# hongsukchoi/Pose2Mesh_RELEASE

Measured on NVIDIA H100. Metric: SMPL meshes/sec, higher is better.
Workload: dtype f32 (wgmma fp16x3 split, fp32 accumulate)

## Files before the change

pose2mesh_release_b200/csrc/cheb_umma.cu:

```cuda
#include <cuda.h>
#include <cuda_fp16.h>
#include <cuda_runtime.h>

#include <algorithm>
#include <cstdlib>
#include <cstring>
#include <vector>

#include "p2m_internal.h"

namespace p2m {

namespace {

constexpr int TILE_M = 128;
constexpr int FC = 32;
constexpr int A_BLOCK_BYTES = TILE_M * 128;
constexpr float W_SCALE = 64.f;
constexpr float W_INV_SCALE = 1.f / 64.f;

struct TileHeader {
  int n_rows;
  int h1;
  int nnz;
// ... 63 lines not shown
}
template <unsigned SLEEP_NS = 200>
__device__ __forceinline__ void mbar_wait_relaxed(uint32_t bar, uint32_t parity, volatile int* abort_flag, int* status,
                                                  int code) {
  if (mbar_try_wait(bar, parity)) return;
  unsigned long long t0 = 0;
  for (unsigned spin = 0;; ++spin) {
#pragma unroll 1
    for (int it = 0; it < 16; ++it) {
      if (mbar_try_wait(bar, parity)) return;
      __nanosleep(SLEEP_NS);
    }
    if (*abort_flag) return;
    if ((spin & 255u) == 255u) {
      const unsigned long long t = global_ns();
      if (t0 == 0) t0 = t;
      else if (t - t0 > MBAR_TIMEOUT_NS) break;
    }
  }
  mbar_timeout(abort_flag, status, code);
}
__device__ __forceinline__ void fence_barrier_init() { asm volatile("fence.mbarrier_init.release.cluster;" ::: "memory"); }
__device__ __forceinline__ void fence_async_proxy() { asm volatile("fence.proxy.async.shared::cta;" ::: "memory"); }

__device__ __forceinline__ void bulk_g2s(uint32_t dst, const void* src, uint32_t bytes, uint32_t bar) {
  asm volatile("cp.async.bulk.shared::cluster.global.mbarrier::complete_tx::bytes [%0], [%1], %2, [%3];" ::"r"(dst),
               "l"(src), "r"(bytes), "r"(bar)
               : "memory");
}
__device__ __forceinline__ void bulk_s2g(void* dst, uint32_t src, uint32_t bytes) {
  asm volatile("cp.async.bulk.global.shared::cta.bulk_group [%0], [%1], %2;" ::"l"(dst), "r"(src), "r"(bytes) : "memory");
}
__device__ __forceinline__ void bulk_commit() { asm volatile("cp.async.bulk.commit_group;" ::: "memory"); }
__device__ __forceinline__ void bulk_wait_read0() { asm volatile("cp.async.bulk.wait_group.read 0;" ::: "memory"); }
__device__ __forceinline__ void bulk_wait0() { asm volatile("cp.async.bulk.wait_group 0;" ::: "memory"); }
__device__ __forceinline__ void cp_async16(uint32_t dst, const void* src) {
  asm volatile("cp.async.cg.shared.global [%0], [%1], 16;" ::"r"(dst), "l"(src) : "memory");
}
__device__ __forceinline__ void cp_async16_zfill(uint32_t dst, const void* src, uint32_t src_bytes) {
  asm volatile("cp.async.cg.shared.global [%0], [%1], 16, %2;" ::"r"(dst), "l"(src), "r"(src_bytes) : "memory");
}
__device__ __forceinline__ void tma_load_2d(uint32_t dst, const CUtensorMap* tm, int c0, int c1, uint32_t bar) {
  asm volatile(
      "cp.async.bulk.tensor.2d.shared::cluster.global.mbarrier::complete_tx::bytes [%0], [%1, {%2, %3}], [%4];" ::"r"(dst),
      "l"(reinterpret_cast<uint64_t>(tm)), "r"(c0), "r"(c1), "r"(bar)
      : "memory");
}
__device__ __forceinline__ void prefetch_l2(const void* ptr) {
  asm volatile("prefetch.global.L2 [%0];" ::"l"(ptr));
}
__device__ __forceinline__ void cp_async_arrive_noinc(uint32_t bar) {
  asm volatile("cp.async.mbarrier.arrive.noinc.shared::cta.b64 [%0];" ::"r"(bar) : "memory");
}
__device__ __forceinline__ void producer_barrier() { asm volatile("bar.sync 1, 512;" ::: "memory"); }
__device__ __forceinline__ float4 lds_f4(uint32_t a) {
  float4 v;
  asm volatile("ld.shared.v4.f32 {%0, %1, %2, %3}, [%4];" : "=f"(v.x), "=f"(v.y), "=f"(v.z), "=f"(v.w) : "r"(a));
  return v;
}
__device__ __forceinline__ float2 lds_f2(uint32_t a) {
  float2 v;
  asm volatile("ld.shared.v2.f32 {%0, %1}, [%2];" : "=f"(v.x), "=f"(v.y) : "r"(a));
  return v;
}
__device__ __forceinline__ uint2 lds_u2(uint32_t a) {
  uint2 v;
  asm volatile("ld.shared.v2.u32 {%0, %1}, [%2];" : "=r"(v.x), "=r"(v.y) : "r"(a));
  return v;
}
__device__ __forceinline__ uint32_t lds_u16(uint32_t a) {
  unsigned short v;
  asm volatile("ld.shared.u16 %0, [%1];" : "=h"(v) : "r"(a));
  return v;
}
__device__ __forceinline__ void sts_f4(uint32_t a, const float4& v) {
  asm volatile("st.shared.v4.f32 [%0], {%1, %2, %3, %4};" ::"r"(a), "f"(v.x), "f"(v.y), "f"(v.z), "f"(v.w) : "memory");
}
__device__ __forceinline__ void sts_f2(uint32_t a, float x, float y) {
  asm volatile("st.shared.v2.f32 [%0], {%1, %2};" ::"r"(a), "f"(x), "f"(y) : "memory");
}
__device__ __forceinline__ void sts_u2(uint32_t a, const uint2& v) {
  asm volatile("st.shared.v2.u32 [%0], {%1, %2};" ::"r"(a), "r"(v.x), "r"(v.y) : "memory");
}
__device__ __forceinline__ void fma4(float4& acc, float w, const float4& x) {
  acc.x = fmaf(w, x.x, acc.x);
  acc.y = fmaf(w, x.y, acc.y);
  acc.z = fmaf(w, x.z, acc.z);
  acc.w = fmaf(w, x.w, acc.w);
}
__device__ __forceinline__ float4 cheb_t2(const float4& g, const float4& x) {
  return make_float4(fmaf(2.f, g.x, -x.x), fmaf(2.f, g.y, -x.y), fmaf(2.f, g.z, -x.z), fmaf(2.f, g.w, -x.w));
}
__device__ __forceinline__ float4 gather_row4(uint32_t ent, uint32_t e, uint32_t e1, uint32_t rows_q) {
  float4 acc0 = make_float4(0.f, 0.f, 0.f, 0.f), acc1 = acc0;
  for (; e + 3 < e1; e += 4) {
    const uint2 a0 = lds_u2(ent + e * 8), a1 = lds_u2(ent + e * 8 + 8), a2 = lds_u2(ent + e * 8 + 16),
                a3 = lds_u2(ent + e * 8 + 24);
    const float4 x0 = lds_f4(rows_q + a0.x), x1 = lds_f4(rows_q + a1.x), x2 = lds_f4(rows_q + a2.x),
                 x3 = lds_f4(rows_q + a3.x);
    fma4(acc0, __uint_as_float(a0.y), x0);
    fma4(acc1, __uint_as_float(a1.y), x1);
    fma4(acc0, __uint_as_float(a2.y), x2);
    fma4(acc1, __uint_as_float(a3.y), x3);
  }
  if (e + 1 < e1) {
    const uint2 a0 = lds_u2(ent + e * 8), a1 = lds_u2(ent + e * 8 + 8);
    const float4 x0 = lds_f4(rows_q + a0.x), x1 = lds_f4(rows_q + a1.x);
// ... 55 lines not shown
};
__device__ __forceinline__ void split4(const float4& v, uint2& hi, uint2& lo) {
  __half2 h0 = __floats2half2_rn(v.x, v.y), h1 = __floats2half2_rn(v.z, v.w);
  float2 f0 = __half22float2(h0), f1 = __half22float2(h1);
  __half2 l0 = __floats2half2_rn(v.x - f0.x, v.y - f0.y), l1 = __floats2half2_rn(v.z - f1.x, v.w - f1.y);
  hi.x = *reinterpret_cast<uint32_t*>(&h0);
  hi.y = *reinterpret_cast<uint32_t*>(&h1);
  lo.x = *reinterpret_cast<uint32_t*>(&l0);
  lo.y = *reinterpret_cast<uint32_t*>(&l1);
}

struct KParams {
  const float* x;
  int in_unpool;
  int V, P, fin;
  int n_tiles;
  const unsigned char* meta;
  const int* meta_bytes;
  int meta_stride, max_h1;
  const unsigned char* wpack;
  const float* zero_row;
  EpiDev ep;
  int res_identity;
  const float* t1;
  const float* a_scale;
  long long ldy;
  int y_col0;
  float* y;
  int* status;
  long long* trace;
  int own_table;
  const float* head_wt;
  float* head_z;
  const unsigned char* apack;
  long long wslice_bytes;
  long long wblock_stride;
  int tma;
  CUtensorMap tm_x, tm_t1;
};

#ifdef P2M_UMMA_TRACE
__device__ __forceinline__ void trace_ev(const KParams& p, int role, int& n, int ev) {
  if (p.trace != nullptr && blockIdx.x == 0 && blockIdx.y == 0 && n < 512) {
    p.trace[role * 512 + n] = ((long long)ev << 48) | (clock64() & 0xFFFFFFFFFFFFll);
    ++n;
  }
}
#else
__device__ __forceinline__ void trace_ev(const KParams&, int, int&, int) {}
#endif

constexpr int W_PROD = 16;
constexpr int W_XLOAD = 16, N_XLOAD = 2, W_BLOAD = 18, W_EPI0 = 20;
constexpr int NUM_THREADS2 = 24 * 32;
constexpr int REGS_LAUNCH = 80, REGS_UTIL = 40, REGS_EPI = 120;
static_assert(128 * (REGS_EPI - REGS_LAUNCH) <= 128 * (REGS_LAUNCH - REGS_UTIL), "register pool balance");
static_assert(W_XLOAD % 4 == 0 && W_EPI0 % 4 == 0 && W_EPI0 - W_XLOAD == 4, "setmaxnreg works on aligned warpgroups");

template <int N>
__host__ __device__ constexpr int tile_rows() { return N == 128 ? 64 : TILE_M; }
template <int N, int NS, int XS, int MODE>
__global__ void __launch_bounds__(NUM_THREADS2, 1) k_cheb_conv_umma(const __grid_constant__ KParams p) {
  static_assert(N == 64 || N == 128, "one warpgroup holds the CTA's 128 x 64 or 64 x 128 accumulator in registers");
  constexpr int TM = tile_rows<N>();
  constexpr int RPT = TM / 64;
  constexpr int H = TM / 64;
  constexpr int ER = 16 * H;
  constexpr bool KT1 = (MODE == 1);
  constexpr bool plain = !KT1;
  constexpr bool XDIRECT = KT1 && NS >= 3;
  constexpr int A_BYTES = TM * 128;
  constexpr int B_BLOCK_BYTES = N * 128;
  constexpr int SLOT_BYTES = A_BYTES + B_BLOCK_BYTES;

  extern __shared__ __align__(1024) unsigned char smem_raw[];
  unsigned char* ring = smem_raw;
  float* Xs = reinterpret_cast<float*>(ring + NS * SLOT_BYTES);
  const size_t xs_stage_floats = (XDIRECT && TM == 64) ? 0 : (size_t)TM * FC;
  float* T1s = Xs + XS * xs_stage_floats;
  const size_t t1_stage_floats = (size_t)p.max_h1 * FC;
  unsigned char* meta_s =
      reinterpret_cast<unsigned char*>(T1s + (plain ? 0 : XS) * t1_stage_floats);
  uint64_t* bars = reinterpret_cast<uint64_t*>(meta_s + 2 * (size_t)p.meta_stride);
  uint64_t* b_ab_full = bars;
  uint64_t* b_ab_empty = b_ab_full + NS;
  uint64_t* b_x_full = b_ab_empty + NS;
  uint64_t* b_x_empty = b_x_full + XS;
  uint64_t* b_m_full = b_x_empty + XS;
  uint64_t* b_m_empty = b_m_full + 2;
  uint32_t* flags = reinterpret_cast<uint32_t*>(b_m_empty + 2);
  volatile int* abort_flag = reinterpret_cast<volatile int*>(flags + 1);
  float* ep_mul = reinterpret_cast<float*>(flags + 4);
  float* ep_add = ep_mul + N;
  constexpr int EC = 32;
  constexpr int STG_WARP_BYTES = N == 128 ? 16 * STG_ROW_BYTES : 32 * EC * 4;
  unsigned char* epi_stage =
      reinterpret_cast<unsigned char*>((reinterpret_cast<uintptr_t>(ep_add + N) + 127) & ~(uintptr_t)127);
  int* own_s = reinterpret_cast<int*>(epi_stage + 4 * STG_WARP_BYTES);
  float* head_w_s = reinterpret_cast<float*>(own_s + 4 * 32);
  uint64_t* b_res = reinterpret_cast<uint64_t*>(head_w_s);

  const int tid = threadIdx.x;
  const int warp = tid >> 5;
  const int lane = tid & 31;
  const int n_chunk = p.fin / FC;
  const int n_use = 3 * n_chunk;

  if (tid == 0) {
    for (int s = 0; s < NS; ++s) {
      mbar_init(smem_u32(b_ab_full + s), p.apack != nullptr ? 1 : W_PROD + 1);
      mbar_init(smem_u32(b_ab_empty + s), 4);
    }
    for (int s = 0; s < XS; ++s) {
      mbar_init(smem_u32(b_x_full + s), N_XLOAD * 32 + 1);
      mbar_init(smem_u32(b_x_empty + s), 1);
    }
    for (int s = 0; s < 2; ++s) {
      mbar_init(smem_u32(b_m_full + s), 1);
      mbar_init(smem_u32(b_m_empty + s), 1);
    }
    if (N == 128)
      for (int w = 0; w < 4; ++w) mbar_init(smem_u32(b_res + w), 1);
    *abort_flag = (smem_u32(ring) & 1023u) ? 1 : 0;
    if (*abort_flag) mbar_timeout(abort_flag, p.status, 100);
    fence_barrier_init();
  }
  const float a_scale = p.a_scale ? *p.a_scale : 1.f;
  const int ecol0 = (int)blockIdx.y * N;
  for (int n = threadIdx.x; n < N; n += NUM_THREADS2) {
    const float sc = (p.ep.scale ? p.ep.scale[ecol0 + n] : 1.f) / a_scale;
    const float sh = p.ep.scale ? p.ep.shift[ecol0 + n] : 0.f;
    const float bi = p.ep.bias ? p.ep.bias[ecol0 + n] : 0.f;
    ep_mul[n] = W_INV_SCALE * sc;
    ep_add[n] = fmaf(bi, p.ep.scale ? p.ep.scale[ecol0 + n] : 1.f, sh);
  }
  if (N == 64 && p.head_z != nullptr)
    for (int i = threadIdx.x; i < 64 * 12; i += NUM_THREADS2) head_w_s[i] = p.head_wt[i];
  __syncthreads();

  if (warp >= W_XLOAD && warp < W_EPI0) {
  asm volatile("setmaxnreg.dec.sync.aligned.u32 %0;" ::"n"(REGS_UTIL));
  if (warp >= W_XLOAD && warp < W_XLOAD + N_XLOAD) {
    if (p.apack == nullptr) {
      const int lt = tid - W_XLOAD * 32;
      const int lq = lt & 7, lrg = lt >> 3;
      const int my_tiles = (p.n_tiles - (int)blockIdx.x + (int)gridDim.x - 1) / (int)gridDim.x;
      if (lt == 32 && p.tma) {
        if (!XDIRECT) asm volatile("prefetch.tensormap [%0];" ::"l"(reinterpret_cast<uint64_t>(&p.tm_x)) : "memory");
        if (KT1) asm volatile("prefetch.tensormap [%0];" ::"l"(reinterpret_cast<uint64_t>(&p.tm_t1)) : "memory");
      }
      auto fetch_meta = [&](int itf) {
        const int pat = (blockIdx.x + itf * gridDim.x) % p.P;
        const int m = itf & 1;
        mbar_wait_relaxed(smem_u32(b_m_empty + m), ((itf >> 1) & 1) ^ 1, abort_flag, p.status, 1);
        const int mbytes = p.meta_bytes[pat];
        mbar_arrive_expect_tx(smem_u32(b_m_full + m), mbytes);
        bulk_g2s(smem_u32(meta_s + (size_t)m * p.meta_stride), p.meta + (size_t)pat * p.meta_stride, mbytes,
                 smem_u32(b_m_full + m));
      };
      if (lt == 0 && my_tiles > 0) fetch_meta(0);
      const uint32_t fin_bytes = (uint32_t)p.fin * 4u;
      const int sh = p.in_unpool ? 1 : 0;
      int g2 = 0;
      int ltn = 0;
      for (int it2 = 0; it2 < my_tiles; ++it2) {
        const int tile2 = blockIdx.x + it2 * gridDim.x;
        const long long mesh_row0 = (long long)(tile2 / p.P) * p.V;
        const int m2 = it2 & 1;
        mbar_wait_relaxed(smem_u32(b_m_full + m2), (it2 >> 1) & 1, abort_flag, p.status, 8);
        const unsigned char* mb2 = meta_s + (size_t)m2 * p.meta_stride;
        const TileHeader* hdr2 = reinterpret_cast<const TileHeader*>(mb2);
        const int* halo = reinterpret_cast<const int*>(mb2 + hdr2->off_halo);
        const int h1 = hdr2->h1;
        for (int c2 = 0; c2 < n_chunk; ++c2, ++g2) {
          const int xs2 = g2 % XS;
          mbar_wait_relaxed(smem_u32(b_x_empty + xs2), ((g2 / XS) & 1) ^ 1, abort_flag, p.status, 11);
          if (lt == 0) trace_ev(p, 4, ltn, 1);
          const uint32_t xbar = smem_u32(b_x_full + xs2);
          auto stage_rows = [&](uint32_t dbase, const char* sbase, int first, int n_rows, int shift) {
            for (int i0 = first + lrg; i0 < n_rows; i0 += 32) {
              int v[4];
#pragma unroll
              for (int u = 0; u < 4; ++u) v[u] = (i0 + 8 * u < n_rows) ? halo[i0 + 8 * u] : -2;
#pragma unroll
              for (int u = 0; u < 4; ++u) {
                if (v[u] != -2) {
                  const uint32_t srow = (uint32_t)max(v[u], 0) >> shift;
                  cp_async16_zfill(dbase + (i0 + 8 * u) * 128, sbase + (uint64_t)srow * (uint64_t)fin_bytes,
                                   v[u] >= 0 ? 16u : 0u);
                }
              }
            }
          };
          const char* t1_mesh =
              reinterpret_cast<const char*>(KT1 ? p.t1 + mesh_row0 * p.fin + c2 * FC + lq * 4 : nullptr);
          const char* x_mesh = reinterpret_cast<const char*>(p.x + (mesh_row0 >> sh) * p.fin + c2 * FC + lq * 4);
          const uint32_t t1_dst = smem_u32(T1s + xs2 * t1_stage_floats) + lq * 16;
          const uint32_t x_dst = smem_u32(Xs + xs2 * xs_stage_floats) + lq * 16;
          if (p.tma) {
            if (lt == 32) {
              const int own0 = tile2 * TM;
              mbar_arrive_expect_tx(xbar, (XDIRECT ? 0 : (p.in_unpool ? TM / 2 : TM) * 128) + (KT1 ? TM * 128 : 0));
              if (!XDIRECT)
                tma_load_2d(smem_u32(Xs + xs2 * xs_stage_floats), &p.tm_x, c2 * FC, p.in_unpool ? own0 >> 1 : own0, xbar);
              if (KT1) tma_load_2d(smem_u32(T1s + xs2 * t1_stage_floats), &p.tm_t1, c2 * FC, own0, xbar);
            }
            if (KT1) stage_rows(t1_dst, t1_mesh, TM, h1, 0);
          } else {
            if (KT1) stage_rows(t1_dst, t1_mesh, 0, h1, 0);
            if (!XDIRECT) stage_rows(x_dst, x_mesh, 0, TM, sh);
            if (lt == 32) mbar_arrive(xbar);
          }
          cp_async_arrive_noinc(xbar);
          if (lt == 0) trace_ev(p, 4, ltn, 2);
          if (lt == 0 && c2 == (n_chunk > 1 ? 1 : 0) && it2 + 1 < my_tiles) fetch_meta(it2 + 1);
        }
      }
    }
  } else if (warp == W_BLOAD) {
    if (lane == 0) {
      uint32_t ucnt = 0;
      int tn = 0;
      const int uses = plain ? n_chunk : n_use;
      for (int tile = blockIdx.x; tile < p.n_tiles; tile += gridDim.x) {
        for (int u = 0; u < uses; ++u, ++ucnt) {
          const int s = ucnt % NS;
          const uint32_t par = (ucnt / NS) & 1;
          mbar_wait_relaxed(smem_u32(b_ab_empty + s), par ^ 1, abort_flag, p.status, 4);
          trace_ev(p, 1, tn, 10 + u);
          const unsigned char* wsl = p.wpack + (size_t)blockIdx.y * (size_t)p.wslice_bytes;
          if (p.apack != nullptr) {
            mbar_arrive_expect_tx(smem_u32(b_ab_full + s), B_BLOCK_BYTES + A_BYTES);
            bulk_g2s(smem_u32(ring + s * SLOT_BYTES), p.apack + ((size_t)tile * uses + u) * A_BYTES, A_BYTES,
                     smem_u32(b_ab_full + s));
          } else {
            mbar_arrive_expect_tx(smem_u32(b_ab_full + s), B_BLOCK_BYTES);
          }
          bulk_g2s(smem_u32(ring + s * SLOT_BYTES + A_BYTES), wsl + (size_t)u * (size_t)p.wblock_stride, B_BLOCK_BYTES,
                   smem_u32(b_ab_full + s));
        }
      }
    }
  }
  } else if (warp >= W_EPI0) {
    asm volatile("setmaxnreg.inc.sync.aligned.u32 %0;" ::"n"(REGS_EPI));
    const int wq = warp - W_EPI0;
    constexpr int CPR = EC / 4;
    constexpr int RPI = 32 / CPR;
    const uint32_t stg = smem_u32(epi_stage) + (uint32_t)wq * STG_WARP_BYTES;
    const int prow = lane / CPR, pc = lane % CPR;
    constexpr int NP = ER / RPI;
    int colk[2];
#pragma unroll
    for (int k = 0; k < 2; ++k) colk[k] = (int)(((uint32_t)pc ^ (uint32_t)((k * RPI + prow) & 7)) << 2);
    const int trow = (lane >> 4) * 64 + wq * 16 + (lane & 15);
    const int uses = plain ? n_chunk : n_use;
    uint32_t ucnt = 0;
    int it = 0;
    int etn = 0;
    for (int tile = blockIdx.x; tile < p.n_tiles; tile += gridDim.x, ++it) {
      const int b = tile / p.P, pat = tile - b * p.P;
      const long long mesh0 = (long long)b * p.V;
      int* own_w = own_s + wq * 32;
      {
        int v;
        if (lane >= ER) {
          v = -1;
        } else if (p.own_table) {
          v = __ldg(reinterpret_cast<const int*>(p.meta + (size_t)pat * p.meta_stride + 64) + trow);
        } else {
          v = pat * TM + trow;
          if (v >= p.V) v = -1;
        }
        __syncwarp();
        own_w[lane] = v;
        __syncwarp();
      }
      int own_v[NP];
#pragma unroll
      for (int i = 0; i < NP; ++i) own_v[i] = own_w[i * RPI + prow];
      if (N == 128) {
        if (lane < ER) bulk_wait_read0();
        __syncwarp();
        if (p.ep.res != nullptr && p.res_identity) {
          const uint32_t rbar = smem_u32(b_res + wq);
          const int n_valid = __popc(__ballot_sync(0xFFFFFFFFu, lane < ER && own_w[lane] >= 0));
          if (lane == 0) mbar_arrive_expect_tx(rbar, (uint32_t)n_valid * (N * 4));
          __syncwarp();
          if (lane < ER && own_w[lane] >= 0) {
            const long long r = mesh0 + own_w[lane];
            bulk_g2s(stg + lane * STG_ROW_BYTES, p.ep.res + (p.ep.res_unpool ? (r >> 1) : r) * p.ep.res_F + ecol0, N * 4,
                     rbar);
          }
        }
      }
      if (p.ep.res != nullptr && (N == 64 || !p.res_identity)) {
        const int lpr = ((p.apack != nullptr ? N : p.ep.res_F) * 4 + 127) >> 7;
        for (int j = lane; j < ER * lpr; j += 32) {
          const int rr = j / lpr, ln = j - rr * lpr;
          const int vtx = own_w[rr];
          if (vtx >= 0) {
            const long long r = mesh0 + vtx;
            prefetch_l2(p.ep.res + (p.ep.res_unpool ? (r >> 1) : r) * p.ep.res_F + (p.apack != nullptr ? ecol0 : 0) + ln * 32);
          }
        }
      }
      float acc[2][32];
#pragma unroll
      for (int h = 0; h < 2; ++h)
#pragma unroll
        for (int j = 0; j < 32; ++j) acc[h][j] = 0.f;
      if (wq == 0 && lane == 0) trace_ev(p, 3, etn, 1);
      for (int u = 0; u < uses; ++u, ++ucnt) {
        const uint32_t s = ucnt % NS;
        if (wq == 0 && lane == 0) trace_ev(p, 3, etn, 4);
        mbar_wait(smem_u32(b_ab_full + s), (ucnt / NS) & 1, abort_flag, p.status, 6);
        if (wq == 0 && lane == 0) trace_ev(p, 3, etn, 5);
        const uint32_t a0 = smem_u32(ring + s * SLOT_BYTES);
        wg_fence();
#pragma unroll
        for (int h = 0; h < 2; ++h) {
          const uint64_t da = make_desc_sw128(a0 + (TM == 128 ? (uint32_t)h * (64 * 128) : 0u));
          const uint64_t db = make_desc_sw128(a0 + A_BYTES + (TM == 64 ? (uint32_t)h * (64 * 128) : 0u));
          wgmma_m64n64<0, 0>(acc[h], da + 0, db + 0);
          wgmma_m64n64<0, 0>(acc[h], da + 2, db + 2);
          wgmma_m64n64<0, 0>(acc[h], da + 4, db + 0);
          wgmma_m64n64<0, 0>(acc[h], da + 6, db + 2);
          wgmma_m64n64<0, 0>(acc[h], da + 0, db + 4);
          wgmma_m64n64<0, 0>(acc[h], da + 2, db + 6);
        }
        wg_commit();
        wg_wait0();
        __syncwarp();
        if (lane == 0) mbar_arrive(smem_u32(b_ab_empty + s));
      }
      if (wq == 0 && lane == 0) trace_ev(p, 3, etn, 2);
      auto stage_slab = [&](int cb) {
#pragma unroll
        for (int h = 0; h < H; ++h)
#pragma unroll
          for (int jj = 0; jj < 4; ++jj)
#pragma unroll
            for (int r = 0; r < 2; ++r) {
              const int lr = 16 * h + (lane >> 2) + 8 * r;
              const int cc = 8 * jj + 2 * (lane & 3);
              const int j = 4 * (cb / 8 + jj) + 2 * r;
              sts_f2(stg + lr * (EC * 4) + ((((uint32_t)(cc >> 2)) ^ (uint32_t)(lr & 7)) << 4) + (cc & 3) * 4,
                     acc[h][j], acc[h][j + 1]);
            }
        __syncwarp();
      };
      if (N == 64 && p.head_z != nullptr) {
        float z[12];
#pragma unroll
        for (int j = 0; j < 12; ++j) z[j] = 0.f;
#pragma unroll
        for (int cb = 0; cb < N; cb += 32) {
          stage_slab(cb);
#pragma unroll
          for (int c = 0; c < 8; ++c) {
            const float4 a = lds_f4(stg + lane * (EC * 4) + (((uint32_t)c ^ (uint32_t)(lane & 7)) << 4));
            const float av[4] = {a.x, a.y, a.z, a.w};
#pragma unroll
            for (int e = 0; e < 4; ++e) {
              const int n = cb + 4 * c + e;
              float t = fmaf(av[e], ep_mul[n], ep_add[n]);
              if (p.ep.relu) t = fmaxf(t, 0.f);
              const float4 w0 = *reinterpret_cast<const float4*>(head_w_s + n * 12);
              const float4 w1 = *reinterpret_cast<const float4*>(head_w_s + n * 12 + 4);
              const float4 w2 = *reinterpret_cast<const float4*>(head_w_s + n * 12 + 8);
              z[0] = fmaf(t, w0.x, z[0]); z[1] = fmaf(t, w0.y, z[1]); z[2] = fmaf(t, w0.z, z[2]); z[3] = fmaf(t, w0.w, z[3]);
              z[4] = fmaf(t, w1.x, z[4]); z[5] = fmaf(t, w1.y, z[5]); z[6] = fmaf(t, w1.z, z[6]); z[7] = fmaf(t, w1.w, z[7]);
              z[8] = fmaf(t, w2.x, z[8]); z[9] = fmaf(t, w2.y, z[9]); z[10] = fmaf(t, w2.z, z[10]); z[11] = fmaf(t, w2.w, z[11]);
            }
          }
          __syncwarp();
        }
        if (own_w[lane] >= 0) {
          float4* zr = reinterpret_cast<float4*>(p.head_z + (mesh0 + own_w[lane]) * 12);
          zr[0] = make_float4(z[0], z[1], z[2], z[3]);
          zr[1] = make_float4(z[4], z[5], z[6], z[7]);
          zr[2] = make_float4(z[8], z[9], z[10], z[11]);
        }
      } else if (N == 128) {
        const bool res_id = p.ep.res != nullptr && p.res_identity;
        if (res_id) mbar_wait(smem_u32(b_res + wq), (uint32_t)it & 1u, abort_flag, p.status, 12);
        if (wq == 0 && lane == 0) trace_ev(p, 3, etn, 21);
#pragma unroll
        for (int h = 0; h < 2; ++h)
#pragma unroll
          for (int jg = 0; jg < 8; ++jg) {
            const int n = 64 * h + 8 * jg + 2 * (lane & 3);
            const float2 mu = *reinterpret_cast<const float2*>(ep_mul + n);
            const float2 ad = *reinterpret_cast<const float2*>(ep_add + n);
#pragma unroll
            for (int r = 0; r < 2; ++r) {
              const int j = 4 * jg + 2 * r;
              const uint32_t a = stg + ((lane >> 2) + 8 * r) * STG_ROW_BYTES + n * 4;
              float o0 = fmaf(acc[h][j], mu.x, ad.x), o1 = fmaf(acc[h][j + 1], mu.y, ad.y);
              if (p.ep.relu) {
                o0 = fmaxf(o0, 0.f);
                o1 = fmaxf(o1, 0.f);
              }
              if (res_id) {
                const float2 rv = lds_f2(a);
                o0 += rv.x;
                o1 += rv.y;
              }
              sts_f2(a, o0, o1);
            }
          }
        if (p.ep.res != nullptr && !p.res_identity) {
          __syncwarp();
          const int gn = ecol0 + 4 * lane;
          for (int rr = 0; rr < ER; ++rr) {
            const int vtx = own_w[rr];
            if (vtx >= 0) {
              const long long r = mesh0 + vtx;
              const float* res_row = p.ep.res + (p.ep.res_unpool ? (r >> 1) : r) * p.ep.res_F;
              const uint32_t a = stg + rr * STG_ROW_BYTES + lane * 16;
              const float4 v = lds_f4(a);
              float o[4] = {v.x, v.y, v.z, v.w};
#pragma unroll
              for (int e = 0; e < 4; ++e) {
                const float l = __ldg(p.ep.lam + gn + e);
                o[e] += (1.f - l) * __ldg(res_row + __ldg(p.ep.i0 + gn + e)) + l * __ldg(res_row + __ldg(p.ep.i1 + gn + e));
              }
              sts_f4(a, make_float4(o[0], o[1], o[2], o[3]));
            }
          }
        }
        if (wq == 0 && lane == 0) trace_ev(p, 3, etn, 22);
        fence_async_proxy();
        __syncwarp();
        if (lane < ER) {
          if (own_w[lane] >= 0)
            bulk_s2g(p.y + (mesh0 + own_w[lane]) * p.ldy + p.y_col0 + ecol0, stg + lane * STG_ROW_BYTES, N * 4);
          bulk_commit();
        }
        if (wq == 0 && lane == 0) trace_ev(p, 3, etn, 23);
      } else {
#pragma unroll
        for (int cb = 0; cb < N; cb += 32) {
          stage_slab(cb);
          float4 mu_k[2], ad_k[2];
#pragma unroll
          for (int k = 0; k < 2; ++k) {
            mu_k[k] = *reinterpret_cast<const float4*>(ep_mul + cb + colk[k]);
            ad_k[k] = *reinterpret_cast<const float4*>(ep_add + cb + colk[k]);
          }
#pragma unroll
          for (int i = 0; i < NP; ++i) {
            const int rr = i * RPI + prow;
            const int n = cb + colk[i & 1];
            const int gn = ecol0 + n;
            const float4 a = lds_f4(stg + rr * (EC * 4) + (pc << 4));
            const int vtx = own_v[i];
            if (vtx >= 0) {
              const float4 mu = mu_k[i & 1], ad = ad_k[i & 1];
              float o[4] = {fmaf(a.x, mu.x, ad.x), fmaf(a.y, mu.y, ad.y), fmaf(a.z, mu.z, ad.z), fmaf(a.w, mu.w, ad.w)};
              if (p.ep.relu) {
#pragma unroll
                for (int e = 0; e < 4; ++e) o[e] = fmaxf(o[e], 0.f);
              }
              const long long r = mesh0 + vtx;
              if (p.ep.res != nullptr) {
                const float* res_row = p.ep.res + (p.ep.res_unpool ? (r >> 1) : r) * p.ep.res_F;
                if (p.res_identity) {
                  const float4 rv = __ldg(reinterpret_cast<const float4*>(res_row + gn));
                  o[0] += rv.x; o[1] += rv.y; o[2] += rv.z; o[3] += rv.w;
                } else {
#pragma unroll
                  for (int e = 0; e < 4; ++e) {
                    const float l = __ldg(p.ep.lam + gn + e);
                    o[e] += (1.f - l) * __ldg(res_row + __ldg(p.ep.i0 + gn + e)) + l * __ldg(res_row + __ldg(p.ep.i1 + gn + e));
                  }
                }
              }
              *reinterpret_cast<float4*>(p.y + r * p.ldy + p.y_col0 + gn) = make_float4(o[0], o[1], o[2], o[3]);
            }
          }
          __syncwarp();
        }
      }
    }
    if (N == 128 && lane < ER) bulk_wait0();
  } else {
    if (p.apack == nullptr) {
    const int q = tid & 7;
    const int rg = tid >> 3;
    const uint32_t t1s_a = smem_u32(T1s);
    const uint32_t ring_a = smem_u32(ring);
    const int my_tiles = (p.n_tiles - (int)blockIdx.x + (int)gridDim.x - 1) / (int)gridDim.x;
    const int n_stage = my_tiles * n_chunk;

    uint32_t row[RPT], re[RPT], ent_a = 0;
    int ptn = 0;
    uint32_t slot = 0, spar = 0;
    uint32_t so_f[RPT], so_s[RPT];
#pragma unroll
    for (int ps = 0; ps < RPT; ++ps) row[ps] = re[ps] = so_f[ps] = so_s[ps] = 0;
    const bool odd = (rg & 1) != 0;
    auto next_slot = [&]() {
      if (++slot == (uint32_t)NS) {
        slot = 0;
        spar ^= 1u;
      }
    };

    const int xsh = (p.tma && p.in_unpool) ? 1 : 0;
    const float* xp[RPT];
#pragma unroll
    for (int ps = 0; ps < RPT; ++ps) xp[ps] = nullptr;
    int it = 0, c = -1;
    for (int g = 0; g < n_stage; ++g) {
      if (++c == n_chunk) {
        c = 0;
        ++it;
      }
      const int m = it & 1;
      const int xs = g % XS;
      float4 xd[RPT];
#pragma unroll
      for (int ps = 0; ps < RPT; ++ps) {
        xd[ps] = make_float4(0.f, 0.f, 0.f, 0.f);
        if (XDIRECT && c != 0 && xp[ps]) xd[ps] = __ldg(reinterpret_cast<const float4*>(xp[ps] + c * FC));
      }
      if (tid == 0) trace_ev(p, 0, ptn, 1);
      mbar_wait(smem_u32(b_x_full + xs), (g / XS) & 1, abort_flag, p.status, 9);
      if (tid == 0) trace_ev(p, 0, ptn, 2);

      if (c == 0) {
        mbar_wait(smem_u32(b_m_full + m), (it >> 1) & 1, abort_flag, p.status, 8);
        const unsigned char* mb = meta_s + (size_t)m * p.meta_stride;
        const TileHeader* hdr = reinterpret_cast<const TileHeader*>(mb);
        const uint32_t mb_a = smem_u32(mb);
        const uint32_t rp_a = mb_a + hdr->off_rp, ord2_a = mb_a + hdr->off_ord2;
        ent_a = mb_a + hdr->off_ent;
#pragma unroll
        for (int ps = 0; ps < RPT; ++ps) {
          row[ps] = plain ? (uint32_t)(64 * ps + rg) : lds_u16(ord2_a + 2 * (64 * ps + rg));
          re[ps] = plain ? 0u : (lds_u16(rp_a + 2 * row[ps]) | (lds_u16(rp_a + 2 * row[ps] + 2) << 16));
          const uint32_t i = row[ps];
          const uint32_t a_hi = sw128_off(i, q >> 1) + (q & 1) * 8, a_lo = sw128_off(i, 4 + (q >> 1)) + (q & 1) * 8;
          so_f[ps] = odd ? a_lo : a_hi;
          so_s[ps] = odd ? a_hi : a_lo;
        }
        if (XDIRECT) {
          const int* halo = reinterpret_cast<const int*>(mb + hdr->off_halo);
          const int sh = p.in_unpool ? 1 : 0;
          const long long mesh_row0 = (long long)((blockIdx.x + (unsigned)it * gridDim.x) / (unsigned)p.P) * p.V;
          const float* xm = p.x + (mesh_row0 >> sh) * p.fin + q * 4;
#pragma unroll
          for (int ps = 0; ps < RPT; ++ps) {
            const int v = halo[row[ps]];
            xp[ps] = (v >= 0) ? xm + (size_t)((uint32_t)v >> sh) * (uint32_t)p.fin : nullptr;
            if (xp[ps]) xd[ps] = __ldg(reinterpret_cast<const float4*>(xp[ps]));
          }
        }
      }
      const uint32_t xs_q = smem_u32(Xs + xs * xs_stage_floats) + q * 16;
      const uint32_t t1s_q = t1s_a + (uint32_t)(xs * t1_stage_floats * 4) + q * 16;
      if (plain) {
        const uint32_t s = slot;
        mbar_wait(smem_u32(b_ab_empty + s), spar ^ 1u, abort_flag, p.status, 10);
        const uint32_t ablk = ring_a + s * SLOT_BYTES;
#pragma unroll
        for (int ps = 0; ps < RPT; ++ps) {
          const uint32_t i = ps * 64 + rg;
          float4 v = lds_f4(xs_q + (i >> xsh) * 128);
          v.x *= a_scale; v.y *= a_scale; v.z *= a_scale; v.w *= a_scale;
          uint2 hi, lo;
          split4(v, hi, lo);
          sts_u2(ablk + so_f[ps], odd ? lo : hi);
          sts_u2(ablk + so_s[ps], odd ? hi : lo);
        }
        fence_async_proxy();
        __syncwarp();
        if ((tid & 31) == 0) mbar_arrive(smem_u32(b_ab_full + s));
        next_slot();
        producer_barrier();
        if (tid == 0) mbar_arrive(smem_u32(b_x_empty + xs));
        if (tid == 0 && c == n_chunk - 1) mbar_arrive(smem_u32(b_m_empty + m));
        continue;
      }
      const uint32_t slot0 = slot;
      auto emit = [&](const float4 (&vv)[RPT]) {
        const uint32_t s = slot;
        if (NS < 3) mbar_wait(smem_u32(b_ab_empty + s), spar ^ 1u, abort_flag, p.status, 10);
        const uint32_t ablk = ring_a + s * SLOT_BYTES;
#pragma unroll
        for (int ps = 0; ps < RPT; ++ps) {
          uint2 hi, lo;
          float4 v = vv[ps];
          if (p.a_scale != nullptr) {
            v.x *= a_scale; v.y *= a_scale; v.z *= a_scale; v.w *= a_scale;
          }
          split4(v, hi, lo);
          sts_u2(ablk + so_f[ps], odd ? lo : hi);
          sts_u2(ablk + so_s[ps], odd ? hi : lo);
        }
        if (NS < 3) {
          fence_async_proxy();
          __syncwarp();
          if ((tid & 31) == 0) mbar_arrive(smem_u32(b_ab_full + s));
        }
        next_slot();
      };
      float4 x[RPT], t1v[RPT], t2[RPT];
      if (NS < 3) {
#pragma unroll
        for (int ps = 0; ps < RPT; ++ps) x[ps] = lds_f4(xs_q + (row[ps] >> xsh) * 128);
        emit(x);
#pragma unroll
        for (int ps = 0; ps < RPT; ++ps) t1v[ps] = lds_f4(t1s_q + row[ps] * 128);
        emit(t1v);
#pragma unroll
        for (int ps = 0; ps < RPT; ++ps) t2[ps] = gather_row4(ent_a, re[ps] & 0xFFFFu, re[ps] >> 16, t1s_q);
        if (tid == 0) trace_ev(p, 0, ptn, 6);
#pragma unroll
        for (int ps = 0; ps < RPT; ++ps) t2[ps] = cheb_t2(t2[ps], x[ps]);
        emit(t2);
      } else {
#pragma unroll
        for (int ps = 0; ps < RPT; ++ps) t2[ps] = gather_row4(ent_a, re[ps] & 0xFFFFu, re[ps] >> 16, t1s_q);
#pragma unroll
        for (int ps = 0; ps < RPT; ++ps) x[ps] = XDIRECT ? xd[ps] : lds_f4(xs_q + (row[ps] >> xsh) * 128);
#pragma unroll
        for (int ps = 0; ps < RPT; ++ps) t1v[ps] = lds_f4(t1s_q + row[ps] * 128);
        if (tid == 0) trace_ev(p, 0, ptn, 6);
        {
          uint32_t s2 = slot + 2, p2 = spar;
          if (s2 >= (uint32_t)NS) {
            s2 -= (uint32_t)NS;
            p2 ^= 1u;
          }
          mbar_wait(smem_u32(b_ab_empty + s2), p2 ^ 1u, abort_flag, p.status, 10);
        }
        emit(x);
        emit(t1v);
#pragma unroll
        for (int ps = 0; ps < RPT; ++ps) t2[ps] = cheb_t2(t2[ps], x[ps]);
        emit(t2);
      }
      if (NS >= 3) {
        fence_async_proxy();
        __syncwarp();
        if ((tid & 31) == 0) {
#pragma unroll
          for (int k = 0; k < 3; ++k) mbar_arrive(smem_u32(b_ab_full + (slot0 + k) % NS));
        }
      }
      if (tid == 0) trace_ev(p, 0, ptn, 7);
      producer_barrier();
      if (tid == 0) trace_ev(p, 0, ptn, 8);
      if (tid == 0) mbar_arrive(smem_u32(b_x_empty + xs));
      if (tid == 0 && c == n_chunk - 1) mbar_arrive(smem_u32(b_m_empty + m));
    }
    }
  }
}

struct DwParams {
  const float* x;
  int in_unpool;
  int V, P, fin;
  int n_tiles;
  const unsigned char* meta;
  const int* meta_bytes;
  int meta_stride, max_h1;
  const float* g;
  int fout_total, m_off, m_cols;
  int chunk0;
  const float* a_scale;
  float* dw;
  int* status;
  const float* t1;
  int g_unpool;
  int swap;
  int tma;
  CUtensorMap tm_x, tm_t1;
};

__device__ __forceinline__ uint64_t make_desc_sw128_mn(uint32_t saddr, uint32_t lbo_bytes) {
  uint64_t d = 0;
  d |= (uint64_t)((saddr & 0x3FFFF) >> 4);
  d |= (uint64_t)((lbo_bytes >> 4) & 0x3FFF) << 16;
  d |= (uint64_t)(1024 >> 4) << 32;
  d |= (uint64_t)1 << 62;
  return d;
}

constexpr int DW_NS = 3;
constexpr int DW_G_BYTES = 4 * A_BLOCK_BYTES;

template <int XS>
__global__ void __launch_bounds__(NUM_THREADS2, 1) k_cheb_dw_umma(const __grid_constant__ DwParams p) {
  extern __shared__ __align__(1024) unsigned char smem_raw[];
  unsigned char* ring = smem_raw;
  unsigned char* gblk = ring + DW_NS * A_BLOCK_BYTES;
  float* Xs = reinterpret_cast<float*>(gblk + DW_G_BYTES);
  constexpr size_t xs_stage_floats = (size_t)TILE_M * FC;
  float* T1s = Xs + XS * xs_stage_floats;
  const size_t t1_stage_floats = (size_t)p.max_h1 * FC;
  unsigned char* meta_s = reinterpret_cast<unsigned char*>(T1s + XS * t1_stage_floats);
  uint64_t* bars = reinterpret_cast<uint64_t*>(meta_s + 2 * (size_t)p.meta_stride);
  uint64_t* b_t_full = bars;
// ... 216 lines not shown
        }
        fence_async_proxy();
        __syncwarp();
        if ((tid & 31) == 0) mbar_arrive(smem_u32(b_g_full));
      }
      for (int c = 0; c < n_chunk; ++c, ++gcnt) {
        const int xs = gcnt % XS;
        mbar_wait(smem_u32(b_x_full + xs), (gcnt / XS) & 1, abort_flag, p.status, 29);
        const uint32_t xs_q = smem_u32(Xs + xs * xs_stage_floats) + q * 16;
        const uint32_t t1s_q = t1s_a + (uint32_t)(xs * t1_stage_floats * 4) + q * 16;
        float4 tv[3][2];
        {
          const float4 g0 = gather_row4(ent_a, r0e & 0xFFFFu, r0e >> 16, t1s_q);
          const float4 g1 = gather_row4(ent_a, r1e & 0xFFFFu, r1e >> 16, t1s_q);
          tv[0][0] = lds_f4(xs_q + row0 * 128);
          tv[0][1] = lds_f4(xs_q + row1 * 128);
          tv[1][0] = lds_f4(t1s_q + row0 * 128);
          tv[1][1] = lds_f4(t1s_q + row1 * 128);
          const float4 a = tv[0][0], c2 = tv[0][1];
          tv[2][0] = cheb_t2(g0, a);
          tv[2][1] = cheb_t2(g1, c2);
          if (p.swap) {
#pragma unroll
            for (int k = 0; k < 3; ++k)
#pragma unroll
              for (int ps = 0; ps < 2; ++ps) {
                tv[k][ps].x *= a_scale; tv[k][ps].y *= a_scale; tv[k][ps].z *= a_scale; tv[k][ps].w *= a_scale;
              }
          }
        }
        const uint32_t u0 = ucnt;
#pragma unroll
        for (int k = 0; k < 3; ++k, ++ucnt) {
          const int s = ucnt % DW_NS;
          mbar_wait(smem_u32(b_t_empty + s), ((ucnt / DW_NS) & 1) ^ 1, abort_flag, p.status, 30);
          const uint32_t blk = ring_a + s * A_BLOCK_BYTES + (q & 1) * 8;
#pragma unroll
          for (int ps = 0; ps < 2; ++ps) {
            const uint32_t i = ps ? row1 : row0;
            uint2 hi, lo;
            split4(tv[k][ps], hi, lo);
            const uint32_t a_hi = blk + sw128_off(i, q >> 1), a_lo = blk + sw128_off(i, 4 + (q >> 1));
            const bool odd = (rg & 1) != 0;
            sts_u2(odd ? a_lo : a_hi, odd ? lo : hi);
            sts_u2(odd ? a_hi : a_lo, odd ? hi : lo);
          }
        }
        fence_async_proxy();
        __syncwarp();
        if ((tid & 31) == 0) {
#pragma unroll
          for (int k = 0; k < 3; ++k) mbar_arrive(smem_u32(b_t_full + (u0 + k) % DW_NS));
        }
        producer_barrier();
        if (tid == 0) {
          mbar_arrive(smem_u32(b_x_empty + xs));
          if (c == n_chunk - 1) mbar_arrive(smem_u32(b_m_empty + m));
        }
      }
    }
  }
}

struct T1Params {
  const float* x;
  int in_unpool;
  int V, P, fin;
  const unsigned char* meta;
  const int* meta_bytes;
  int meta_stride, max_h1;
  float* t1;
};

template <int T1_STAGES>
__global__ void __launch_bounds__(512, 2) k_cheb_t1(const T1Params p) {
  extern __shared__ __align__(16) unsigned char smem_t1[];
  unsigned char* meta_s = smem_t1;
  float* Xs = reinterpret_cast<float*>(smem_t1 + p.meta_stride);
  const size_t stage_floats = (size_t)p.max_h1 * FC;
  const int tid = threadIdx.x, q = tid & 7, rg = tid >> 3;
  const int tile = blockIdx.x;
  const int b = tile / p.P, pat = tile - b * p.P;
  const long long mesh_row0 = (long long)b * p.V;
  {
    const uint4* src = reinterpret_cast<const uint4*>(p.meta + (size_t)pat * p.meta_stride);
    uint4* dst = reinterpret_cast<uint4*>(meta_s);
    const int n16 = p.meta_bytes[pat] >> 4;
    for (int i = tid; i < n16; i += 512) dst[i] = src[i];
  }
  __syncthreads();
  const TileHeader* hdr = reinterpret_cast<const TileHeader*>(meta_s);
  const int h1 = hdr->h1;
  const int* halo = reinterpret_cast<const int*>(meta_s + hdr->off_halo);
  const uint32_t mb_a = smem_u32(meta_s);
  const uint32_t rp_a = mb_a + hdr->off_rp, ent_a = mb_a + hdr->off_ent, ord2_a = mb_a + hdr->off_ord2;
  const int n_chunk = p.fin / FC;
  long long srow[4];
#pragma unroll
  for (int u = 0; u < 4; ++u) {
    const int i = rg + 64 * u;
    const int v = (i < h1) ? halo[i] : -2;
    long long r = mesh_row0 + v;
    if (p.in_unpool) r >>= 1;
    srow[u] = (v >= 0) ? r * p.fin : (long long)v;
  }
  auto stage = [&](int c) {
    if (c < n_chunk) {
// ... 582 lines not shown
```

Measured before the change: 11690.

## Add second MMA/epilogue warpgroup for N=128 to ping-pong tiles

For the N=128 configuration, the producer shrinks to 8 warps and warps 8-11 become a second MMA/epilogue warpgroup. The two warpgroups alternate tiles and are serialized on the MMA phase through a turn barrier, so one group's epilogue overlaps the other's MMA. A staging-free barrier guards the shared epilogue stage, and the residual bulk load moves after the MMA. Register budgets are rebalanced with setmaxnreg, and warps 12-15 are parked at a low register count. The cost is fewer producer threads and extra barrier handshakes.

```diff
diff --git a/pose2mesh_release_b200/csrc/cheb_umma.cu b/pose2mesh_release_b200/csrc/cheb_umma.cu
--- a/pose2mesh_release_b200/csrc/cheb_umma.cu
+++ b/pose2mesh_release_b200/csrc/cheb_umma.cu
@@ -139,7 +139,8 @@
 __device__ __forceinline__ void cp_async_arrive_noinc(uint32_t bar) {
   asm volatile("cp.async.mbarrier.arrive.noinc.shared::cta.b64 [%0];" ::"r"(bar) : "memory");
 }
-__device__ __forceinline__ void producer_barrier() { asm volatile("bar.sync 1, 512;" ::: "memory"); }
+template <int NT>
+__device__ __forceinline__ void producer_barrier() { asm volatile("bar.sync 1, %0;" ::"n"(NT) : "memory"); }
 __device__ __forceinline__ float4 lds_f4(uint32_t a) {
   float4 v;
   asm volatile("ld.shared.v4.f32 {%0, %1, %2, %3}, [%4];" : "=f"(v.x), "=f"(v.y), "=f"(v.z), "=f"(v.w) : "r"(a));
@@ -301,10 +302,18 @@
 
 constexpr int W_PROD = 16;
 constexpr int W_XLOAD = 16, N_XLOAD = 2, W_BLOAD = 18, W_EPI0 = 20;
+constexpr int W_EPI1 = 8, W_PARK = 12;
 constexpr int NUM_THREADS2 = 24 * 32;
 constexpr int REGS_LAUNCH = 80, REGS_UTIL = 40, REGS_EPI = 120;
+constexpr int REGS_PROD2 = 88, REGS_PARK = 24;
 static_assert(128 * (REGS_EPI - REGS_LAUNCH) <= 128 * (REGS_LAUNCH - REGS_UTIL), "register pool balance");
+static_assert(2 * 128 * (REGS_PROD2 - REGS_LAUNCH) + 2 * 128 * (REGS_EPI - REGS_LAUNCH) <=
+                  128 * (REGS_LAUNCH - REGS_PARK) + 128 * (REGS_LAUNCH - REGS_UTIL),
+              "register pool balance of the N = 128 layout");
 static_assert(W_XLOAD % 4 == 0 && W_EPI0 % 4 == 0 && W_EPI0 - W_XLOAD == 4, "setmaxnreg works on aligned warpgroups");
+static_assert(W_EPI1 % 4 == 0 && W_PARK == W_EPI1 + 4 && W_XLOAD == W_PARK + 4, "setmaxnreg works on aligned warpgroups");
+template <int N>
+__host__ __device__ constexpr int prod_warps() { return N == 128 ? W_EPI1 : W_PROD; }
 
 template <int N>
 __host__ __device__ constexpr int tile_rows() { return N == 128 ? 64 : TILE_M; }
@@ -312,7 +321,11 @@
 __global__ void __launch_bounds__(NUM_THREADS2, 1) k_cheb_conv_umma(const __grid_constant__ KParams p) {
   static_assert(N == 64 || N == 128, "one warpgroup holds the CTA's 128 x 64 or 64 x 128 accumulator in registers");
   constexpr int TM = tile_rows<N>();
-  constexpr int RPT = TM / 64;
+  constexpr int NPW = prod_warps<N>();
+  constexpr int NRG = NPW * 4;
+  constexpr int RPT = TM / NRG;
+  constexpr int NWG = N == 128 ? 2 : 1;
+  static_assert(RPT == 2, "both configurations give a producer thread two tile rows");
   constexpr int H = TM / 64;
   constexpr int ER = 16 * H;
   constexpr bool KT1 = (MODE == 1);
@@ -337,7 +350,9 @@
   uint64_t* b_x_empty = b_x_full + XS;
   uint64_t* b_m_full = b_x_empty + XS;
   uint64_t* b_m_empty = b_m_full + 2;
-  uint32_t* flags = reinterpret_cast<uint32_t*>(b_m_empty + 2);
+  uint64_t* b_stg_free = b_m_empty + 2;
+  uint64_t* b_turn = b_stg_free + 1;
+  uint32_t* flags = reinterpret_cast<uint32_t*>(b_turn + 1);
   volatile int* abort_flag = reinterpret_cast<volatile int*>(flags + 1);
   float* ep_mul = reinterpret_cast<float*>(flags + 4);
   float* ep_add = ep_mul + N;
@@ -346,7 +361,7 @@
   unsigned char* epi_stage =
       reinterpret_cast<unsigned char*>((reinterpret_cast<uintptr_t>(ep_add + N) + 127) & ~(uintptr_t)127);
   int* own_s = reinterpret_cast<int*>(epi_stage + 4 * STG_WARP_BYTES);
-  float* head_w_s = reinterpret_cast<float*>(own_s + 4 * 32);
+  float* head_w_s = reinterpret_cast<float*>(own_s + NWG * 4 * ER);
   uint64_t* b_res = reinterpret_cast<uint64_t*>(head_w_s);
 
   const int tid = threadIdx.x;
@@ -357,7 +372,7 @@
 
   if (tid == 0) {
     for (int s = 0; s < NS; ++s) {
-      mbar_init(smem_u32(b_ab_full + s), p.apack != nullptr ? 1 : W_PROD + 1);
+      mbar_init(smem_u32(b_ab_full + s), p.apack != nullptr ? 1 : NPW + 1);
       mbar_init(smem_u32(b_ab_empty + s), 4);
     }
     for (int s = 0; s < XS; ++s) {
@@ -368,8 +383,11 @@
       mbar_init(smem_u32(b_m_full + s), 1);
       mbar_init(smem_u32(b_m_empty + s), 1);
     }
-    if (N == 128)
+    if (N == 128) {
       for (int w = 0; w < 4; ++w) mbar_init(smem_u32(b_res + w), 1);
+      mbar_init(smem_u32(b_stg_free), 4);
+      mbar_init(smem_u32(b_turn), 4);
+    }
     *abort_flag = (smem_u32(ring) & 1023u) ? 1 : 0;
     if (*abort_flag) mbar_timeout(abort_flag, p.status, 100);
     fence_barrier_init();
@@ -387,6 +405,7 @@
     for (int i = threadIdx.x; i < 64 * 12; i += NUM_THREADS2) head_w_s[i] = p.head_wt[i];
   __syncthreads();
 
+  const int mma_g = warp >= W_EPI0 ? 0 : (NWG == 2 && warp >= W_EPI1 && warp < W_PARK) ? 1 : -1;
   if (warp >= W_XLOAD && warp < W_EPI0) {
   asm volatile("setmaxnreg.dec.sync.aligned.u32 %0;" ::"n"(REGS_UTIL));
   if (warp >= W_XLOAD && warp < W_XLOAD + N_XLOAD) {
@@ -491,9 +510,11 @@
       }
     }
   }
-  } else if (warp >= W_EPI0) {
+  } else if (mma_g >= 0) {
     asm volatile("setmaxnreg.inc.sync.aligned.u32 %0;" ::"n"(REGS_EPI));
-    const int wq = warp - W_EPI0;
+    const int g = mma_g;
+    const int wq = warp - (g == 0 ? W_EPI0 : W_EPI1);
+    const int tr = 3 + 2 * g;
     constexpr int CPR = EC / 4;
     constexpr int RPI = 32 / CPR;
     const uint32_t stg = smem_u32(epi_stage) + (uint32_t)wq * STG_WARP_BYTES;
@@ -504,13 +525,12 @@
     for (int k = 0; k < 2; ++k) colk[k] = (int)(((uint32_t)pc ^ (uint32_t)((k * RPI + prow) & 7)) << 2);
     const int trow = (lane >> 4) * 64 + wq * 16 + (lane & 15);
     const int uses = plain ? n_chunk : n_use;
-    uint32_t ucnt = 0;
-    int it = 0;
     int etn = 0;
-    for (int tile = blockIdx.x; tile < p.n_tiles; tile += gridDim.x, ++it) {
+    for (int it = g; (int)blockIdx.x + it * (int)gridDim.x < p.n_tiles; it += NWG) {
+      const int tile = blockIdx.x + it * gridDim.x;
       const int b = tile / p.P, pat = tile - b * p.P;
       const long long mesh0 = (long long)b * p.V;
-      int* own_w = own_s + wq * 32;
+      int* own_w = own_s + (g * 4 + wq) * ER;
       {
         int v;
         if (lane >= ER) {
@@ -522,35 +542,21 @@
           if (v >= p.V) v = -1;
         }
         __syncwarp();
-        own_w[lane] = v;
+        if (lane < ER) own_w[lane] = v;
         __syncwarp();
       }
       int own_v[NP];
 #pragma unroll
       for (int i = 0; i < NP; ++i) own_v[i] = own_w[i * RPI + prow];
-      if (N == 128) {
-        if (lane < ER) bulk_wait_read0();
-        __syncwarp();
-        if (p.ep.res != nullptr && p.res_identity) {
-          const uint32_t rbar = smem_u32(b_res + wq);
-          const int n_valid = __popc(__ballot_sync(0xFFFFFFFFu, lane < ER && own_w[lane] >= 0));
-          if (lane == 0) mbar_arrive_expect_tx(rbar, (uint32_t)n_valid * (N * 4));
-          __syncwarp();
-          if (lane < ER && own_w[lane] >= 0) {
-            const long long r = mesh0 + own_w[lane];
-            bulk_g2s(stg + lane * STG_ROW_BYTES, p.ep.res + (p.ep.res_unpool ? (r >> 1) : r) * p.ep.res_F + ecol0, N * 4,
-                     rbar);
-          }
-        }
-      }
-      if (p.ep.res != nullptr && (N == 64 || !p.res_identity)) {
-        const int lpr = ((p.apack != nullptr ? N : p.ep.res_F) * 4 + 127) >> 7;
+      if (p.ep.res != nullptr) {
+        const bool own_cols = p.apack != nullptr || (N == 128 && p.res_identity);
+        const int lpr = ((own_cols ? N : p.ep.res_F) * 4 + 127) >> 7;
         for (int j = lane; j < ER * lpr; j += 32) {
           const int rr = j / lpr, ln = j - rr * lpr;
           const int vtx = own_w[rr];
           if (vtx >= 0) {
             const long long r = mesh0 + vtx;
-            prefetch_l2(p.ep.res + (p.ep.res_unpool ? (r >> 1) : r) * p.ep.res_F + (p.apack != nullptr ? ecol0 : 0) + ln * 32);
+            prefetch_l2(p.ep.res + (p.ep.res_unpool ? (r >> 1) : r) * p.ep.res_F + (own_cols ? ecol0 : 0) + ln * 32);
           }
         }
       }
@@ -559,12 +565,17 @@
       for (int h = 0; h < 2; ++h)
 #pragma unroll
         for (int j = 0; j < 32; ++j) acc[h][j] = 0.f;
-      if (wq == 0 && lane == 0) trace_ev(p, 3, etn, 1);
+      if (wq == 0 && lane == 0) trace_ev(p, tr, etn, 1);
+      if (NWG == 2 && it > 0) {
+        mbar_wait(smem_u32(b_turn), (uint32_t)(it - 1) & 1u, abort_flag, p.status, 13);
+        if (wq == 0 && lane == 0) trace_ev(p, tr, etn, 3);
+      }
+      uint32_t ucnt = (uint32_t)it * (uint32_t)uses;
       for (int u = 0; u < uses; ++u, ++ucnt) {
         const uint32_t s = ucnt % NS;
-        if (wq == 0 && lane == 0) trace_ev(p, 3, etn, 4);
+        if (wq == 0 && lane == 0) trace_ev(p, tr, etn, 4);
         mbar_wait(smem_u32(b_ab_full + s), (ucnt / NS) & 1, abort_flag, p.status, 6);
-        if (wq == 0 && lane == 0) trace_ev(p, 3, etn, 5);
+        if (wq == 0 && lane == 0) trace_ev(p, tr, etn, 5);
         const uint32_t a0 = smem_u32(ring + s * SLOT_BYTES);
         wg_fence();
 #pragma unroll
@@ -583,7 +594,8 @@
         __syncwarp();
         if (lane == 0) mbar_arrive(smem_u32(b_ab_empty + s));
       }
-      if (wq == 0 && lane == 0) trace_ev(p, 3, etn, 2);
+      if (NWG == 2 && lane == 0) mbar_arrive(smem_u32(b_turn));
+      if (wq == 0 && lane == 0) trace_ev(p, tr, etn, 2);
       auto stage_slab = [&](int cb) {
 #pragma unroll
         for (int h = 0; h < H; ++h)
@@ -632,9 +644,22 @@
           zr[2] = make_float4(z[8], z[9], z[10], z[11]);
         }
       } else if (N == 128) {
+        if (it > 0) mbar_wait(smem_u32(b_stg_free), (uint32_t)(it - 1) & 1u, abort_flag, p.status, 14);
+        if (wq == 0 && lane == 0) trace_ev(p, tr, etn, 20);
         const bool res_id = p.ep.res != nullptr && p.res_identity;
-        if (res_id) mbar_wait(smem_u32(b_res + wq), (uint32_t)it & 1u, abort_flag, p.status, 12);
-        if (wq == 0 && lane == 0) trace_ev(p, 3, etn, 21);
+        if (res_id) {
+          const uint32_t rbar = smem_u32(b_res + wq);
+          const int n_valid = __popc(__ballot_sync(0xFFFFFFFFu, lane < ER && own_w[lane] >= 0));
+          if (lane == 0) mbar_arrive_expect_tx(rbar, (uint32_t)n_valid * (N * 4));
+          __syncwarp();
+          if (lane < ER && own_w[lane] >= 0) {
+            const long long r = mesh0 + own_w[lane];
+            bulk_g2s(stg + lane * STG_ROW_BYTES, p.ep.res + (p.ep.res_unpool ? (r >> 1) : r) * p.ep.res_F + ecol0, N * 4,
+                     rbar);
+          }
+          mbar_wait(rbar, (uint32_t)it & 1u, abort_flag, p.status, 12);
+        }
+        if (wq == 0 && lane == 0) trace_ev(p, tr, etn, 21);
 #pragma unroll
         for (int h = 0; h < 2; ++h)
 #pragma unroll
@@ -679,7 +704,7 @@
             }
           }
         }
-        if (wq == 0 && lane == 0) trace_ev(p, 3, etn, 22);
+        if (wq == 0 && lane == 0) trace_ev(p, tr, etn, 22);
         fence_async_proxy();
         __syncwarp();
         if (lane < ER) {
@@ -687,7 +712,11 @@
             bulk_s2g(p.y + (mesh0 + own_w[lane]) * p.ldy + p.y_col0 + ecol0, stg + lane * STG_ROW_BYTES, N * 4);
           bulk_commit();
         }
-        if (wq == 0 && lane == 0) trace_ev(p, 3, etn, 23);
+        if (wq == 0 && lane == 0) trace_ev(p, tr, etn, 23);
+        if (lane < ER) bulk_wait_read0();
+        __syncwarp();
+        if (lane == 0) mbar_arrive(smem_u32(b_stg_free));
+        if (wq == 0 && lane == 0) trace_ev(p, tr, etn, 24);
       } else {
 #pragma unroll
         for (int cb = 0; cb < N; cb += 32) {
@@ -734,7 +763,10 @@
       }
     }
     if (N == 128 && lane < ER) bulk_wait0();
+  } else if (warp >= NPW) {
+    asm volatile("setmaxnreg.dec.sync.aligned.u32 %0;" ::"n"(REGS_PARK));
   } else {
+    if (NPW != W_PROD) asm volatile("setmaxnreg.inc.sync.aligned.u32 %0;" ::"n"(REGS_PROD2));
     if (p.apack == nullptr) {
     const int q = tid & 7;
     const int rg = tid >> 3;
@@ -788,7 +820,7 @@
         ent_a = mb_a + hdr->off_ent;
 #pragma unroll
         for (int ps = 0; ps < RPT; ++ps) {
-          row[ps] = plain ? (uint32_t)(64 * ps + rg) : lds_u16(ord2_a + 2 * (64 * ps + rg));
+          row[ps] = plain ? (uint32_t)(NRG * ps + rg) : lds_u16(ord2_a + 2 * (NRG * ps + rg));
           re[ps] = plain ? 0u : (lds_u16(rp_a + 2 * row[ps]) | (lds_u16(rp_a + 2 * row[ps] + 2) << 16));
           const uint32_t i = row[ps];
           const uint32_t a_hi = sw128_off(i, q >> 1) + (q & 1) * 8, a_lo = sw128_off(i, 4 + (q >> 1)) + (q & 1) * 8;
@@ -816,7 +848,7 @@
         const uint32_t ablk = ring_a + s * SLOT_BYTES;
 #pragma unroll
         for (int ps = 0; ps < RPT; ++ps) {
-          const uint32_t i = ps * 64 + rg;
+          const uint32_t i = ps * NRG + rg;
           float4 v = lds_f4(xs_q + (i >> xsh) * 128);
           v.x *= a_scale; v.y *= a_scale; v.z *= a_scale; v.w *= a_scale;
           uint2 hi, lo;
@@ -828,7 +860,7 @@
         __syncwarp();
         if ((tid & 31) == 0) mbar_arrive(smem_u32(b_ab_full + s));
         next_slot();
-        producer_barrier();
+        producer_barrier<NPW * 32>();
         if (tid == 0) mbar_arrive(smem_u32(b_x_empty + xs));
         if (tid == 0 && c == n_chunk - 1) mbar_arrive(smem_u32(b_m_empty + m));
         continue;
@@ -901,7 +933,7 @@
         }
       }
       if (tid == 0) trace_ev(p, 0, ptn, 7);
-      producer_barrier();
+      producer_barrier<NPW * 32>();
       if (tid == 0) trace_ev(p, 0, ptn, 8);
       if (tid == 0) mbar_arrive(smem_u32(b_x_empty + xs));
       if (tid == 0 && c == n_chunk - 1) mbar_arrive(smem_u32(b_m_empty + m));
@@ -1224,7 +1256,7 @@
 #pragma unroll
           for (int k = 0; k < 3; ++k) mbar_arrive(smem_u32(b_t_full + (u0 + k) % DW_NS));
         }
-        producer_barrier();
+        producer_barrier<W_PROD * 32>();
         if (tid == 0) {
           mbar_arrive(smem_u32(b_x_empty + xs));
           if (c == n_chunk - 1) mbar_arrive(smem_u32(b_m_empty + m));
```

Result: faster. 12150, median of 6 (+4.0%).
